# poyentung/ebsd-vae

Measured on AMD Instinct MI355X. Metric: EBSD patterns/sec (128x128, fwd+bwd), higher is better.
Workload: dtype fp32 I/O, f16x3 split MFMA; 1 GPU; c2: VariationalAutoEncoderRawData 128x128, latent 16, batch 256/GPU, fwd+loss+bwd+Adam; global_batch=256, image_size=128, latent_dim=16, parallelism=dp1

## Files before the change

### ebsd-vae_amd/csrc/conv_split.hip

```cpp
#include "conv_common.h"
#include "instnorm_fin.h"

#include <stdlib.h>
#include <type_traits>

namespace ev {

static_assert(NP_F16 == EBSDVAE_PIECES_F16, "piece-format id");

#ifdef EV_PIPE_TRACE
__device__ unsigned long long ev_pipe_trace[4096 * 8 * 6];
#define EV_T(x) unsigned long long x = __builtin_amdgcn_s_memtime()
#define EV_TACC(acc, t0) acc += __builtin_amdgcn_s_memtime() - t0
#else
#define EV_T(x)
#define EV_TACC(acc, t0)
#endif


typedef __bf16 bf16x8 __attribute__((ext_vector_type(8)));
typedef __bf16 bf16x4 __attribute__((ext_vector_type(4)));

constexpr int XCK = 8;
constexpr int ACT_FIRST = 5;
// ... 268 lines not shown

EV_DEVINL void pipe_barrier_lds() {
  asm volatile("" ::: "memory");
  __builtin_amdgcn_s_waitcnt(0xF | (7 << 4) | (3 << 14));
  __builtin_amdgcn_s_barrier();
  asm volatile("" ::: "memory");
}

template <int N>
EV_DEVINL void pipe_barrier() {
  static_assert(N >= 0 && N < 16, "vmcnt range");
  asm volatile("" ::: "memory");
  __builtin_amdgcn_s_waitcnt(N | (7 << 4));
  __builtin_amdgcn_s_barrier();
  asm volatile("" ::: "memory");
}

#ifndef EV_EPI_POL
#define EV_EPI_POL 2
#endif
constexpr int kEpiPol = EV_EPI_POL;

template <int MF, int NF, int FP>
constexpr bool pipe_prefetch_ok() { return NF == 1 && (FP == P_ID || FP == FP_UPSUM); }
template <int MF, int NF, int FP>
constexpr int pipe_prefetch_n() {
  return pipe_prefetch_ok<MF, NF, FP>() ? (FP == FP_UPSUM ? 8 * (MF / 2) : 16 * MF) : 1;
}
template <int MF, int NF, int FP, int NT, int PH = 0>
EV_DEVINL void pipe_epilogue(f32x16 (&acc)[MF][NF], const float* __restrict__ bias,
                             float* __restrict__ y, float2* __restrict__ spart, int H, int W, int b0,
                             int h0, int wpx0, int mfs, int slot, int co_base, int hk, int l32,
                             const float* __restrict__ yprev, const float2* __restrict__ stprev,
                             double2* __restrict__ ipart, float* __restrict__ ypool, float sc,
                             float (&pv)[pipe_prefetch_n<MF, NF, FP>()]) {
  static_assert(MF % 2 == 0, "fragments in 64-pixel pairs");
  static_assert(PH == 0 || pipe_prefetch_ok<MF, NF, FP>(), "prefetch phases: NF 1, P_ID / UPSUM");
  constexpr int NG = MF / 2;
  constexpr bool FUSED = FP == P_ID || FP == P_POOL || FP == P_UP || FP == FP_UPSUM;
#ifndef EV_EPI_OPAQUE
#define EV_EPI_OPAQUE 1
#endif
  constexpr bool EPI_OPAQUE = EV_EPI_OPAQUE && FP == FP_POOLOUT;
  if constexpr (PH == 1) {
    const int nf = 0;
    const int co = co_base + l32;
    if constexpr (FP == FP_UPSUM) {
      const int W2 = W >> 1;
      const auto rp = __builtin_amdgcn_make_buffer_rsrc(
          (void*)(yprev + ((size_t)b0 * (H >> 1) + (h0 >> 1)) * W2 * NT), 0, 0x7fffffff, 0x00020000);
#pragma unroll
      for (int g = 0; g < NG; ++g) {
        const int m0 = 2 * g;
#pragma unroll
        for (int k = 0; k < 8; ++k) {
// ... 80 lines not shown
            gs[k] = (acc[m0][nf][r] + acc[m0][nf][r + 1]) + (acc[m0 + 1][nf][r] + acc[m0 + 1][nf][r + 1]);
            prow = (wpx0 / W + m0) >> 1;
            pc = ((wpx0 % W + 4 * hk) >> 1) + (((r & 3) + 8 * (r >> 2)) >> 1);
          } else {
            const int mf = m0 + (k >> 2), r = 2 * (k & 3);
            gs[k] = (acc[mf][nf][r] + acc[mf][nf][r + 1]) + (acc[mf][nf][r + 8] + acc[mf][nf][r + 9]);
            prow = (wpx0 + mf * mfs) / W >> 1;
            pc = ((r & 3) + 8 * (r >> 2) + 4 * hk) >> 1;
          }
          off[k] = ((prow * W2 + pc) * NT + co) * 4;
        }
#pragma unroll
        for (int k = 0; k < 8; ++k)
          v[k] = PH == 2 ? pv[g * 8 + k]
                         : __builtin_bit_cast(float, __builtin_amdgcn_raw_buffer_load_b32(rp, off[k], 0, kEpiPol));
        float s1 = 0.f, s2 = 0.f;
#pragma unroll
        for (int k = 0; k < 8; ++k) {
          const float h = inbwd_acc<P_ID>(gs[k], &v[k], sp, spc, s1, s2);
          __builtin_amdgcn_raw_buffer_store_b32(__builtin_bit_cast(unsigned, h), rq, off[k], 0, kEpiPol);
        }
        s1 += __shfl_xor(s1, 32, 64);
        s2 += __shfl_xor(s2, 32, 64);
        if (hk == 0) ipart[((size_t)b0 * T + slot + g) * NT + co] = make_double2((double)s1, (double)s2);
      }
    }
    if (FP == FP_POOLOUT) {
      const int W2 = W >> 1;
      const auto rq = __builtin_amdgcn_make_buffer_rsrc(
          (void*)(ypool + ((size_t)b0 * (H >> 1) + (h0 >> 1)) * W2 * NT), 0, 0x7fffffff, 0x00020000);
#pragma unroll
      for (int m0 = 0; m0 < MF; m0 += 2) {
        if (W >= 32) {
          const int prow = (wpx0 / W + m0) >> 1, pcol = (wpx0 % W + 4 * hk) >> 1;
          int pb = ((prow * W2 + pcol) * NT + co) * 4;
          if constexpr (EPI_OPAQUE) asm volatile("" : "+v"(pb));
#pragma unroll
          for (int r = 0; r < 16; r += 2) {
            const float m = fmaxf(fmaxf(acc[m0][nf][r], acc[m0][nf][r + 1]),
                                  fmaxf(acc[m0 + 1][nf][r], acc[m0 + 1][nf][r + 1]));
            const int dc = ((r & 3) + 8 * (r >> 2)) >> 1;
            __builtin_amdgcn_raw_buffer_store_b32(__builtin_bit_cast(unsigned, m), rq,
                                                  pb + dc * NT * 4, 0, kEpiPol);
          }
        } else {
#pragma unroll
          for (int mf = m0; mf < m0 + 2; ++mf) {
// ... 28 lines not shown
#pragma unroll
        for (int e0 = 32 * g; e0 < 32 * g + 32; e0 += G) {
          float v[G][NL];
#pragma unroll
          for (int j = 0; j < G; ++j) {
            const int e = e0 + j, mf = e >> 4, r = e & 15;
            const int pl = pbase + mf * 32 + (r & 3) + 8 * (r >> 2);
#pragma unroll
            for (int k = 0; k < NL; ++k)
              v[j][k] = PH == 2 ? pv[e]
                                : __builtin_bit_cast(float, __builtin_amdgcn_raw_buffer_load_b32(
                                                                rp, (inbwd_pix<FP>(pl, W, lW, k) * NT + co) * 4, 0, kEpiPol));
          }
#pragma unroll
          for (int j = 0; j < G; ++j) {
            const int e = e0 + j, mf = e >> 4, r = e & 15;
            const float h = inbwd_acc<FP>(acc[mf][nf][r], v[j], sp, spc, s1, s2);
            __builtin_amdgcn_raw_buffer_store_b32(__builtin_bit_cast(unsigned, h), ry,
                                                  vbase + (mf * mfs + (r & 3) + 8 * (r >> 2)) * NT * 4, 0, kEpiPol);
          }
        }
        s1 += __shfl_xor(s1, 32, 64);
        s2 += __shfl_xor(s2, 32, 64);
        if (hk == 0) ipart[((size_t)b0 * T + slot + g) * NT + co] = make_double2((double)s1, (double)s2);
      }
    }
    if (!FUSED && spart) {
#pragma unroll
      for (int g = 0; g < NG; ++g) {
        float sg = s[g];
        sg += __shfl_xor(sg, 32, 64);
        const float mean = sg * (1.0f / 64);
        float q = 0.f;
#pragma unroll
        for (int mf = 2 * g; mf < 2 * g + 2; ++mf)
#pragma unroll
          for (int r = 0; r < 16; ++r) {
            const float d = acc[mf][nf][r] - mean;
            q = fmaf(d, d, q);
          }
        q += __shfl_xor(q, 32, 64);
        if (hk == 0) spart[((size_t)b0 * T + slot + g) * NT + co] = make_float2(mean, q);
      }
    }
  }
}

#ifndef EV_WREG
#define EV_WREG 1
#endif
constexpr bool pipe_wreg(int NWV, int WM, int NF, int NI, int WR) {
  return EV_WREG && NWV == 4 && WM == 1 && NF == 1 && NI == 1 && WR == 0;
}

template <int NP, int NWV, int WM, int MF, int NF, int KX, int MODE, int FP, int NI, int WR>
__global__ __launch_bounds__(NWV * 64, (MODE == ACT_FIRST || pipe_wreg(NWV, WM, NF, NI, WR)) ? 1 : 2) void conv3x3_pipe_kernel(
    const float* __restrict__ src, const float2* __restrict__ sstats, const char* __restrict__ wp,
    const float* __restrict__ bias, float* __restrict__ y, float2* __restrict__ spart,
    float* __restrict__ act_out, int B, int H, int W, int Cin, int TH, int tpb,
    const float* __restrict__ yprev, const float2* __restrict__ stprev, double2* __restrict__ ipart,
    float* __restrict__ ypool, const float* __restrict__ gmax, int gmT, float2* __restrict__ st_out,
    float2* __restrict__ bst_out, double fin_inv_hw, const float* __restrict__ w0,
    const float* __restrict__ b0) {
  constexpr int WN = NWV / WM;
  constexpr int NT = WN * NF * 32;
// ... 15 lines not shown
  static_assert(!FIRST || (WR > 0 && NI == 1), "ACT_FIRST: the resident-weight single-image form");
  extern __shared__ __attribute__((aligned(16))) char xsm[];
  const int HP = TH + 2, WP = W + 2;
  const int pixI = HP * WP;
  const int pixP = NI * pixI;
  const int xslab = (pixP + 1) * XPS;
  char* lw0 = xsm;
  char* lx0 = xsm + (WR ? WR * WSLAB : 2 * WSLABP);
  const int XTS = FIRST ? (TH + 4) * (W + 2) : 0;
  float* xtl = reinterpret_cast<float*>(lx0 + 2 * xslab);
  const float4* wtab = reinterpret_cast<const float4*>(xtl + 2 * XTS);

  const int tid = threadIdx.x, lane = tid & 63, wave = tid >> 6;
  const int wm = wave % WM, wn = wave / WM;
  const int l32 = lane & 31, hk = lane >> 5;
  const int tpi = H / TH;
  const int tpx = TH * W;
  const int nch = Cin / XCK;
  const int t0 = blockIdx.x * tpb;
  const int ntl = min(tpb, ((B + NI - 1) / NI) * tpi - t0);
  const int nit = ntl * nch;

  int fpx0 = wm * MW, mfs = 32;
  if ((FP == FP_POOLOUT || FP == FP_UPSUM) && W >= 32) {
    const int cbs = W >> 5, rp = wm / cbs;
    fpx0 = MF * rp * W + (wm - rp * cbs) * 32;
    mfs = W;
  }
  int abase[MF];
#pragma unroll
  for (int mf = 0; mf < MF; ++mf) {
    const int p = fpx0 + mf * mfs + l32;
    const int im = p / tpx, pr = p - im * tpx;
    const int r = pr / W, c = pr - r * W;
    abase[mf] = im * pixI + r * WP + c;
  }
  int toff[5];
#pragma unroll
  for (int s = 0; s < 5; ++s) {
    const int t = min(2 * s + hk, 8);
    toff[s] = (t / 3) * WP + t % 3;
  }

  const int Hs = POOL ? 2 * H : (UPS ? H / 2 : H);
  const int Ws = POOL ? 2 * W : (UPS ? W / 2 : W);
  const int q = tid & 1;
  constexpr int WPI = NWV / NI;
  static_assert(NWV % NI == 0, "waves split evenly over the tile's images");
  const int img_w = wave / WPI;
  const int tig = tid - img_w * WPI * 64;
// ... 227 lines not shown
    }
  };

  f32x16 acc[MF][NF];
  auto zero_acc = [&]() EV_LAMBDA_INLINE {
#pragma unroll
    for (int mf = 0; mf < MF; ++mf)
#pragma unroll
      for (int nf = 0; nf < NF; ++nf)
#pragma unroll
        for (int r = 0; r < 16; ++r) acc[mf][nf][r] = 0.f;
  };
  const int ncol = wn * NF * 32 + l32;
#ifdef EV_PIPE_NOPREF
  constexpr bool PREF = false;
#else
  constexpr bool PREF = pipe_prefetch_ok<MF, NF, FP>() && NI == 1;
#endif
  float pv[pipe_prefetch_n<MF, NF, FP>()];
  auto epi_prefetch = [&](int it) EV_LAMBDA_INLINE {
    int b0, h0, ch;
    coords(it, b0, h0, ch);
    pipe_epilogue<MF, NF, FP, NT, PREF ? 1 : 0>(acc, bias, y, spart, H, W, b0, h0, fpx0, mfs, 0,
                                                wn * NF * 32, hk, l32, yprev, stprev, ipart, ypool, 1.f, pv);
  };
  auto epilogue = [&](int it_done, f32x16 (&ea)[MF][NF]) EV_LAMBDA_INLINE {
    int b0, h0, ch;
    coords(it_done, b0, h0, ch);
    const int im = NI == 1 ? 0 : (wm * MW) / tpx;
    const int wpx0 = fpx0 - im * tpx;
    float sc = 1.f;
    if constexpr (NP == NP_F16) {
      sc = ldexpf(1.f, -wshift);
      if constexpr (GS) sc = ldexpf(sc, -gshift(min(b0 + im, B - 1)));
    }
#ifdef EV_PIPE_NOEPI
    if (sc == 12345.f)
#else
    if (NI == 1 || b0 + im < B)
#endif
      pipe_epilogue<MF, NF, FP, NT, PREF ? 2 : 0>(ea, bias, y, spart, H, W, b0 + im, h0, wpx0, mfs,
                                                  (h0 * W + wm * MW - im * tpx) / 64, wn * NF * 32, hk,
                                                  l32, yprev, stprev, ipart, ypool, sc, pv);
  };

#ifdef EV_PIPE_TRACE
  unsigned long long tr_issue = 0, tr_k = 0, tr_bar = 0, tr_epi = 0;
  const unsigned long long tr_start = __builtin_amdgcn_s_memtime();
  const unsigned long long tr_rstart = __builtin_amdgcn_s_memrealtime();
#endif
  auto body = [&](int it, auto P_c) EV_LAMBDA_INLINE {
    constexpr int P = decltype(P_c)::value;
    constexpr int SL_LD = PD == 2 ? P : 0;
    constexpr int SL_ST = PD == 2 ? 1 - P : 0;
    EV_T(tb0);
    const int it1 = min(it + 1, nit - 1), itp = min(it + PD, nit - 1);
    if constexpr (PREF && P == 1)
      if ((it & (nch - 1)) == nch - 1) epi_prefetch(it);
#ifndef EV_PIPE_LATE_ISSUE
    issue_weights(it1, lw0 + (1 - P) * WSLABP);
    if constexpr (WREG) issue_wreg(it1, std::integral_constant<int, WREG ? 1 - P : 0>());
    issue_halo(itp, std::integral_constant<int, SL_LD>());
#endif
    EV_TACC(tr_issue, tb0);
    EV_T(tb1);
// ... 168 lines not shown
      if (item_live(k)) stage_item(std::integral_constant<int, 0>(), k, fs, lx0);
    stage_post(std::integral_constant<int, 0>(), fs, lx0);
  }
  if constexpr (WR) {
    asm volatile("s_waitcnt vmcnt(%0)" ::"n"(NLD) : "memory");
  }
  __syncthreads();
  for (int tl = 0; tl < ntl; ++tl) {
    for (int ch = 0; ch < nch; ch += 2) {
      body(tl * nch + ch, std::integral_constant<int, 0>());
      body(tl * nch + ch + 1, std::integral_constant<int, 1>());
    }
    EV_T(te0);
    epilogue(tl * nch, acc);
    zero_acc();
    EV_TACC(tr_epi, te0);
  }
  if (st_out || bst_out) {
    asm volatile("s_waitcnt vmcnt(0)" ::: "memory");
    __threadfence_block();
    __syncthreads();
    const int tpi = NI == 1 ? H / TH : 1;
    const int g0 = t0 / tpi, g1 = (t0 + ntl - 1) / tpi;
    for (int gi = g0; gi <= g1; ++gi)
      for (int im = 0; im < NI; ++im) {
        const int b = gi * NI + im;
        if (b >= B) break;
        if (st_out)
          in_stats_finalize_image(spart, st_out, NT, (H * W) / 64, 64.f, b, tid,
                                  reinterpret_cast<float*>(xsm));
        if (bst_out)
          in_bwd_finalize_image(ipart, bst_out, NT, (H * W) / 64, fin_inv_hw, b, tid,
                                reinterpret_cast<double*>(xsm));
      }
  }
#ifdef EV_PIPE_TRACE
  if (lane == 0 && blockIdx.x < 4096) {
    unsigned long long* o = ev_pipe_trace + ((size_t)blockIdx.x * 8 + (wave & 7)) * 6;
    o[0] = __builtin_amdgcn_s_memtime() - tr_start;
    o[1] = tr_issue; o[2] = tr_k; o[3] = tr_bar; o[4] = tr_epi;
    o[5] = __builtin_amdgcn_s_memrealtime() - tr_rstart;
  }
#endif
}

__global__ __launch_bounds__(256) void pack_wmax_kernel(const PackBatch pb) {
  const ebsdvae_pack_desc& q = pb.d[blockIdx.y];
  const int n = q.cin * q.cout * 9;
  float m = 0.f;
  for (int i = blockIdx.x * 256 + threadIdx.x; i < n; i += kF16MaxParts * 256) m = fmaxf(m, fabsf(q.src[i]));
  for (int off = 32; off > 0; off >>= 1) m = fmaxf(m, __shfl_xor(m, off));
  __shared__ float wm[4];
  if ((threadIdx.x & 63) == 0) wm[threadIdx.x >> 6] = m;
  __syncthreads();
  if (threadIdx.x == 0) {
// ... 66 lines not shown
  static const bool v = [] {
    const char* e = getenv("EBSDVAE_CONV_SMALL1");
    return !(e && e[0] == '0');
  }();
  return v;
}

static bool use_multi_image() {
  static const int v = [] {
    const char* e = getenv("EBSDVAE_CONV_MULTI_IMAGE");
    return (e && e[0] == '0') ? 0 : 1;
  }();
  return v != 0;
}

static bool use_wres() {
  static const bool v = [] {
    const char* e = getenv("EBSDVAE_WRES");
    return !(e && e[0] == '0');
  }();
  return v;
}

static int cu_count(hipStream_t s) {
  if (const int n = evh::stream_cus(s)) return n;
  static int cache[64] = {0};
  int dev = 0;
  (void)hipGetDevice(&dev);
  if (dev < 0 || dev >= 64) dev = 0;
  if (!cache[dev]) {
    int n = 0;
    if (hipDeviceGetAttribute(&n, hipDeviceAttributeMultiprocessorCount, dev) != hipSuccess || n <= 0) n = 256;
    cache[dev] = n;
  }
  return cache[dev];
}

struct X3Cfg {
  int M, TH, NT, KX, nwv;
  int NI;
  int wr;
  size_t lds;
  size_t lds_pipe;
};

static bool plan_split(int H, int W, int cin, int cout, int np, X3Cfg* c) {
  if ((np != 2 && np != 3 && np != NP_F16) || cin % (2 * XCK) || !(cout == 128 || cout == 64 || cout == 32)) return false;
  if (np == NP_F16 && !use_pipe()) return false;
  auto pow2 = [](int v) { return v > 0 && (v & (v - 1)) == 0; };
  if (!pow2(cin / XCK) || !pow2(H) || !pow2(W)) return false;
  if (!ev_buf_bytes_ok(4LL * H * W * (cin > cout ? cin : cout) * 4)) return false;
  c->M = (np != 2 && cout != 128) ? 512 : 256;
  c->NI = 1;
  c->NT = cout;
  c->nwv = (cout == 128 || np != 2) ? 8 : 4;
  if (H * W < c->M) {
    if (!((np == 3 || np == NP_F16) && cout == 128 && H * W == 64 && use_pipe() && use_multi_image()))
      return false;
    c->M = 128;
    c->NI = 2;
    c->TH = H;
    if (np == NP_F16 && use_small_one_image()) {
      c->M = 64;
      c->NI = 1;
      c->nwv = 4;
    }
  } else {
    if (W > c->M || c->M % W) return false;
    c->TH = c->M / W;
    if (H % c->TH) return false;
  }
  const int pixI = (c->TH + 2) * (W + 2);
  const int pix = c->NI * pixI;
  const int tpg = (c->nwv / c->NI) * 64;
  c->KX = use_pipe() ? ((c->TH + 2) * W * 2 + tpg - 1) / tpg : (pixI * 2 + tpg - 1) / tpg;
  const int kxmax = np == 2 ? (cout == 128 ? 2 : (cout == 64 ? 5 : 7))
                            : (np == NP_F16 ? (cout == 128 ? 2 : (cout == 64 ? 3 : 4))
                                            : (cout == 128 ? 2 : (cout == 64 ? 4 : 5)));
  if (c->KX > kxmax) return false;
  const int wslab = XTAPS * npc(np) * cout * 16;
  c->lds = 2 * (size_t)wslab + 2 * (size_t)(pix + 1) * XPS;
  c->lds_pipe = 2 * (size_t)pipe_dma_per(wslab, c->nwv) * c->nwv * 1024 + 2 * (size_t)(pix + 1) * XPS;
  if (c->lds_pipe > 160 * 1024) c->lds_pipe = 0;
  c->wr = 0;
  const size_t lds_wr = 4 * (size_t)wslab + 2 * (size_t)(pix + 1) * XPS;
  if (np == NP_F16 && cin == 4 * XCK && c->NI == 1 && use_wres() && use_pipe() && lds_wr <= 160 * 1024) {
    c->wr = 4;
    c->lds_pipe = lds_wr;
  }
  if (c->NI > 1 || np == NP_F16) return c->lds_pipe != 0;
  return c->lds <= 160 * 1024;
}

static bool pipe_owns_images(const X3Cfg& c, int B, int H, hipStream_t s) {
  static const bool on = [] {
    const char* e = getenv("EBSDVAE_FUSE_FINALIZE");
    return !(e && e[0] == '0');
  }();
  if (!on || !(c.NI > 1 || (use_pipe() && c.lds_pipe))) return false;
  const int tpi = c.NI > 1 ? 1 : H / c.TH;
  const int ntiles = ((B + c.NI - 1) / c.NI) * tpi;
  const int ncu = cu_count(s);
  const int tpb = (ntiles + ncu - 1) / ncu;
  return tpb % tpi == 0;
}

static size_t first_lds_extra(int TH, int W) {
  return (2 * (size_t)(TH + 4) * (W + 2) + FIRST_WTAB) * sizeof(float);
}
// ... 38 lines not shown
                      const float* bias, float* y, float* part, float* aout, int B, int H, int W,
                      int cin, hipStream_t s, int pmode, const InBwdFuse& f) {
  if (pmode >= 0) {
    switch (pmode) {
      case P_ID: launch_x3_1<NP, NWV, WM, MF, NF, KX, ACT_RAW, P_ID, NI, WR>(c, src, nullptr, wp, nullptr, y, nullptr, nullptr, B, H, W, cin, s, f); break;
      case P_POOL: launch_x3_1<NP, NWV, WM, MF, NF, KX, ACT_RAW, P_POOL, NI, WR>(c, src, nullptr, wp, nullptr, y, nullptr, nullptr, B, H, W, cin, s, f); break;
      case P_UPSUM:
        if constexpr (NI == 1)
          launch_x3_1<NP, NWV, WM, MF, NF, KX, ACT_RAW, FP_UPSUM, NI, WR>(c, src, nullptr, wp, nullptr, y, nullptr, nullptr, B, H, W, cin, s, f);
        break;
      default: launch_x3_1<NP, NWV, WM, MF, NF, KX, ACT_RAW, P_UP, NI, WR>(c, src, nullptr, wp, nullptr, y, nullptr, nullptr, B, H, W, cin, s, f); break;
    }
    return;
  }
  if constexpr (NI == 1) {
    if (f.ypool) {
      launch_x3_1<NP, NWV, WM, MF, NF, KX, ACT_NORM, FP_POOLOUT, NI, WR>(c, src, st, wp, bias, y, part, aout, B, H, W, cin, s, f);
      return;
    }
  }
  switch (mode) {
    case ACT_RAW: launch_x3_1<NP, NWV, WM, MF, NF, KX, ACT_RAW, FP_NONE, NI, WR>(c, src, st, wp, bias, y, part, aout, B, H, W, cin, s, f); break;
    case ACT_NORM: launch_x3_1<NP, NWV, WM, MF, NF, KX, ACT_NORM, FP_NONE, NI, WR>(c, src, st, wp, bias, y, part, aout, B, H, W, cin, s, f); break;
    case ACT_NORM_POOL: launch_x3_1<NP, NWV, WM, MF, NF, KX, ACT_NORM_POOL, FP_NONE, NI, 0>(c, src, st, wp, bias, y, part, aout, B, H, W, cin, s, f); break;
    case ACT_UP: launch_x3_1<NP, NWV, WM, MF, NF, KX, ACT_UP, FP_NONE, NI, WR>(c, src, st, wp, bias, y, part, aout, B, H, W, cin, s, f); break;
    default: launch_x3_1<NP, NWV, WM, MF, NF, KX, ACT_NORM_UP, FP_NONE, NI, WR>(c, src, st, wp, bias, y, part, aout, B, H, W, cin, s, f); break;
  }
}

static void dispatch_split(const X3Cfg& c, int np, const float* src, const float* st, int mode,
                           const void* wp, const float* bias, float* y, float* part, float* aout,
                           int B, int H, int W, int cin, int cout, hipStream_t s, int pmode,
                           const InBwdFuse& f) {
  if (np == 2) {
    if (cout == 128)
      launch_x3<2, 8, 4, 2, 2, 2>(c, src, st, mode, wp, bias, y, part, aout, B, H, W, cin, s, pmode, f);
    else if (cout == 64)
      launch_x3<2, 4, 4, 2, 2, 5>(c, src, st, mode, wp, bias, y, part, aout, B, H, W, cin, s, pmode, f);
    else
      launch_x3<2, 4, 4, 2, 1, 7>(c, src, st, mode, wp, bias, y, part, aout, B, H, W, cin, s, pmode, f);
  } else if (np == NP_F16) {
    if (cout == 128 && c.NI > 1)
      launch_x3<NP_F16, 8, 2, 2, 1, 1, 2>(c, src, st, mode, wp, bias, y, part, aout, B, H, W, cin, s, pmode, f);
    else if (cout == 128 && c.M == 64)
      launch_x3<NP_F16, 4, 1, 2, 1, 1>(c, src, st, mode, wp, bias, y, part, aout, B, H, W, cin, s, pmode, f);
    else if (cout == 128)
      launch_x3<NP_F16, 8, 4, 2, 2, 2>(c, src, st, mode, wp, bias, y, part, aout, B, H, W, cin, s, pmode, f);
    else if (cout == 64 && c.wr)
      launch_x3<NP_F16, 8, 8, 2, 2, 3, 1, 4>(c, src, st, mode, wp, bias, y, part, aout, B, H, W, cin, s, pmode, f);
    else if (cout == 64)
      launch_x3<NP_F16, 8, 8, 2, 2, 3>(c, src, st, mode, wp, bias, y, part, aout, B, H, W, cin, s, pmode, f);
    else if (c.KX <= 3 && c.wr)
      launch_x3<NP_F16, 8, 8, 2, 1, 3, 1, 4>(c, src, st, mode, wp, bias, y, part, aout, B, H, W, cin, s, pmode, f);
    else if (c.KX <= 3)
      launch_x3<NP_F16, 8, 8, 2, 1, 3>(c, src, st, mode, wp, bias, y, part, aout, B, H, W, cin, s, pmode, f);
    else if (c.wr)
      launch_x3<NP_F16, 8, 8, 2, 1, 4, 1, 4>(c, src, st, mode, wp, bias, y, part, aout, B, H, W, cin, s, pmode, f);
    else
      launch_x3<NP_F16, 8, 8, 2, 1, 4>(c, src, st, mode, wp, bias, y, part, aout, B, H, W, cin, s, pmode, f);
  } else {
    if (cout == 128 && c.NI > 1)
      launch_x3<3, 8, 2, 2, 1, 1, 2>(c, src, st, mode, wp, bias, y, part, aout, B, H, W, cin, s, pmode, f);
    else if (cout == 128)
      launch_x3<3, 8, 4, 2, 2, 2>(c, src, st, mode, wp, bias, y, part, aout, B, H, W, cin, s, pmode, f);
    else if (cout == 64)
      launch_x3<3, 8, 8, 2, 2, 4>(c, src, st, mode, wp, bias, y, part, aout, B, H, W, cin, s, pmode, f);
    else
      launch_x3<3, 8, 8, 2, 1, 5>(c, src, st, mode, wp, bias, y, part, aout, B, H, W, cin, s, pmode, f);
  }
}

}

using namespace ev;

#ifdef EV_PIPE_TRACE
extern "C" int ebsdvae_debug_pipe_trace(void* host, size_t bytes) {
  if (bytes > sizeof(ev_pipe_trace)) bytes = sizeof(ev_pipe_trace);
  return hipMemcpyFromSymbol(host, HIP_SYMBOL(ev_pipe_trace), bytes, 0, hipMemcpyDeviceToHost) == hipSuccess ? 0 : 1;
}
#endif

extern "C" int ebsdvae_conv3x3_split_supported(int H, int W, int cin, int cout, int pieces) {
  X3Cfg c;
  return plan_split(H, W, cin, cout, pieces, &c) ? 1 : 0;
}

extern "C" int ebsdvae_conv3x3_split_stat_tiles(int H, int W, int cout) {
  (void)cout;
  if (!ev_dim_ok(H) || !ev_dim_ok(W)) return -1;
  return (H * W) / 64;
}

extern "C" size_t ebsdvae_pack_split_bytes(int cin, int cout, int pieces) {
  if (cin <= 0 || cout <= 0 || !(pieces == 2 || pieces == 3 || pieces == NP_F16)) return 0;
  return (size_t)(cin / XCK) * XTAPS * npc(pieces) * cout * XCK * 2 +
         (pieces == NP_F16 ? kF16PackTrailer : 0);
}

extern "C" int ebsdvae_pack_conv_weights_split(const ebsdvae_pack_desc* descs, int n, int pieces,
                                               ebsdvae_stream_t stream) {
  EV_REQUIRE(descs && n > 0 && n <= EBSDVAE_MAX_PACK, "pack_conv_weights_split: n=%d out of range", n);
  EV_REQUIRE(pieces == 2 || pieces == 3 || pieces == NP_F16,
             "pack_conv_weights_split: pieces=%d (2, 3 or %d)", pieces, NP_F16);
  PackBatch pb;
// ... 4 lines not shown
    EV_REQUIRE(q.src && q.dst && q.cin > 0 && q.cout > 0 && (q.kind == 0 || q.kind == 1) && ci_ % XCK == 0,
               "pack_conv_weights_split: bad descriptor %d", i);
    pb.d[i] = q;
    const int e = (ci_ / XCK) * XTAPS * (q.for_dgrad ? q.cin : q.cout) * XCK;
    if (e > maxn) maxn = e;
  }
  int bx = (maxn + 255) / 256;
  if (bx > 64) bx = 64;
  if (pieces == NP_F16)
    hipLaunchKernelGGL(pack_wmax_kernel, dim3(kF16MaxParts, n), dim3(256), 0, (hipStream_t)stream, pb);
  hipLaunchKernelGGL(pack_split_kernel, dim3(bx, n), dim3(256), 0, (hipStream_t)stream, pb, pieces);
  return evh::check_launch("pack_conv_weights_split");
}

extern "C" int ebsdvae_conv3x3_fwd_split(const float* src, const float* src_stats, int src_mode,
                                         const void* wpack, const float* bias, float* y,
                                         float* stat_part, float* act_out, int B, int H, int W,
                                         int cin, int cout, int pieces, ebsdvae_stream_t stream) {
  X3Cfg c;
  EV_REQUIRE(src && wpack && y && B > 0, "conv3x3_fwd_split: null pointer or empty batch");
  EV_REQUIRE(src_mode >= 0 && src_mode <= 4, "conv3x3_fwd_split: bad src_mode %d", src_mode);
  EV_REQUIRE(src_mode == ACT_RAW || src_mode == ACT_UP || src_stats,
             "conv3x3_fwd_split: NORM modes need src_stats");
  EV_REQUIRE(plan_split(H, W, cin, cout, pieces, &c),
             "conv3x3_fwd_split: unsupported shape H=%d W=%d cin=%d cout=%d pieces=%d", H, W, cin, cout,
             pieces);
  dispatch_split(c, pieces, src, src_stats, src_mode, wpack, bias, y, stat_part, act_out, B, H, W,
                 cin, cout, (hipStream_t)stream, -1, InBwdFuse());
  return evh::check_launch("conv3x3_fwd_split");
}

extern "C" int ebsdvae_conv3x3_split_pool_ok(int H, int W, int cin, int cout, int pieces) {
  X3Cfg c;
  return (plan_split(H, W, cin, cout, pieces, &c) && use_pipe() && c.lds_pipe && c.NI == 1 &&
          c.TH % 2 == 0 && W >= 16 && (W & (W - 1)) == 0) ? 1 : 0;
}

extern "C" int ebsdvae_conv3x3_fwd_split_pooled(const float* src, const float* src_stats,
                                                int src_mode, const void* wpack, const float* bias,
                                                float* y, float* ypool, float* stat_part, int B,
                                                int H, int W, int cin, int cout, int pieces,
                                                ebsdvae_stream_t stream) {
  X3Cfg c;
  EV_REQUIRE(src && src_stats && wpack && y && ypool && stat_part && B > 0,
             "conv3x3_fwd_split_pooled: null pointer or empty batch");
  EV_REQUIRE(src_mode == ACT_NORM, "conv3x3_fwd_split_pooled: src_mode %d (ACT_NORM only)", src_mode);
  EV_REQUIRE(ebsdvae_conv3x3_split_pool_ok(H, W, cin, cout, pieces) && plan_split(H, W, cin, cout, pieces, &c),
             "conv3x3_fwd_split_pooled: unsupported shape H=%d W=%d cin=%d cout=%d pieces=%d", H, W,
             cin, cout, pieces);
  InBwdFuse f;
  f.ypool = ypool;
  dispatch_split(c, pieces, src, src_stats, src_mode, wpack, bias, y, stat_part, nullptr, B, H, W,
                 cin, cout, (hipStream_t)stream, -1, f);
  return evh::check_launch("conv3x3_fwd_split_pooled");
}

extern "C" int ebsdvae_conv3x3_dgrad_inbwd_split(const float* g, const void* wpack, float* gin,
                                                 const float* y_prev, const float* st_prev,
                                                 int pmode, double* part, int B, int H, int W,
                                                 int cin, int cout, int pieces,
                                                 ebsdvae_stream_t stream) {
  X3Cfg c;
  EV_REQUIRE(g && wpack && gin && B > 0, "conv3x3_dgrad_inbwd_split: null pointer or empty batch");
  EV_REQUIRE(pieces != NP_F16, "conv3x3_dgrad_inbwd_split: fp16 pieces need the gradient scale "
             "(ebsdvae_conv3x3_dgrad_inbwd_f16)");
  EV_REQUIRE(pmode >= -1 && pmode <= P_UPSUM, "conv3x3_dgrad_inbwd_split: bad pmode %d", pmode);
  EV_REQUIRE(pmode != P_UPSUM || ebsdvae_conv3x3_split_pool_ok(H, W, cin, cout, pieces),
             "conv3x3_dgrad_inbwd_split: summed upsample adjoint unsupported for H=%d W=%d", H, W);
  EV_REQUIRE(pmode < 0 || (y_prev && st_prev && part && (W & (W - 1)) == 0),
             "conv3x3_dgrad_inbwd_split: fused reduce needs y_prev, st_prev, part and W = 2^k");
// ... 2 lines not shown
             cin, cout, pieces);
  InBwdFuse f;
  f.yprev = y_prev;
  f.stprev = (const float2*)st_prev;
  f.part = (double2*)part;
  dispatch_split(c, pieces, g, nullptr, ACT_RAW, wpack, nullptr, gin, nullptr, nullptr, B, H, W, cin,
                 cout, (hipStream_t)stream, pmode, f);
  return evh::check_launch("conv3x3_dgrad_inbwd_split");
}

extern "C" int ebsdvae_conv3x3_dgrad_inbwd_f16(const float* g, const float* gmax, int gm_tiles,
                                               const void* wpack, float* gin, const float* y_prev,
                                               const float* st_prev, int pmode, double* part, int B,
                                               int H, int W, int cin, int cout,
                                               ebsdvae_stream_t stream) {
  X3Cfg c;
  EV_REQUIRE(g && gmax && gm_tiles > 0 && wpack && gin && B > 0,
             "conv3x3_dgrad_inbwd_f16: null pointer, empty batch or no gradient maxima");
  EV_REQUIRE(pmode >= -1 && pmode <= P_UPSUM, "conv3x3_dgrad_inbwd_f16: bad pmode %d", pmode);
  EV_REQUIRE(pmode != P_UPSUM || ebsdvae_conv3x3_split_pool_ok(H, W, cin, cout, NP_F16),
             "conv3x3_dgrad_inbwd_f16: summed upsample adjoint unsupported for H=%d W=%d", H, W);
  EV_REQUIRE(pmode < 0 || (y_prev && st_prev && part && (W & (W - 1)) == 0),
             "conv3x3_dgrad_inbwd_f16: fused reduce needs y_prev, st_prev, part and W = 2^k");
  EV_REQUIRE(plan_split(H, W, cin, cout, NP_F16, &c),
             "conv3x3_dgrad_inbwd_f16: unsupported shape H=%d W=%d cin=%d cout=%d", H, W, cin, cout);
  InBwdFuse f;
  f.yprev = y_prev;
  f.stprev = (const float2*)st_prev;
  f.part = (double2*)part;
  f.gmax = gmax;
  f.gmT = gm_tiles;
  dispatch_split(c, NP_F16, g, nullptr, ACT_RAW, wpack, nullptr, gin, nullptr, nullptr, B, H, W, cin,
                 cout, (hipStream_t)stream, pmode, f);
  return evh::check_launch("conv3x3_dgrad_inbwd_f16");
}

extern "C" int ebsdvae_conv3x3_fwd_split_st(const float* src, const float* src_stats, int src_mode,
                                            const void* wpack, const float* bias, float* y,
                                            float* ypool, float* stat_part, float* st, int B,
                                            int H, int W, int cin, int cout, int pieces,
                                            ebsdvae_stream_t stream) {
  X3Cfg c;
  EV_REQUIRE(src && wpack && (y || ypool) && stat_part && st && B > 0,
             "conv3x3_fwd_split_st: null pointer or empty batch");
  EV_REQUIRE(src_mode >= 0 && src_mode <= 4, "conv3x3_fwd_split_st: bad src_mode %d", src_mode);
  EV_REQUIRE(src_mode == ACT_RAW || src_mode == ACT_UP || src_stats,
             "conv3x3_fwd_split_st: NORM modes need src_stats");
  EV_REQUIRE(!ypool || (src_mode == ACT_NORM && ebsdvae_conv3x3_split_pool_ok(H, W, cin, cout, pieces)),
             "conv3x3_fwd_split_st: pooled output unsupported for H=%d W=%d src_mode=%d", H, W, src_mode);
  EV_REQUIRE(plan_split(H, W, cin, cout, pieces, &c),
             "conv3x3_fwd_split_st: unsupported shape H=%d W=%d cin=%d cout=%d pieces=%d", H, W, cin,
             cout, pieces);
  const bool fused = pipe_owns_images(c, B, H, (hipStream_t)stream);
  InBwdFuse f;
  f.ypool = ypool;
  if (fused) f.st_out = (float2*)st;
  dispatch_split(c, pieces, src, src_stats, src_mode, wpack, bias, y, stat_part, nullptr, B, H, W,
                 cin, cout, (hipStream_t)stream, -1, f);
  if (int rc = evh::check_launch("conv3x3_fwd_split_st")) return rc;
  if (fused) return 0;
  const int T = ebsdvae_conv3x3_split_stat_tiles(H, W, cout);
  return ebsdvae_in_stats_finalize(stat_part, st, B, cout, T, (H * W) / T, stream);
}

extern "C" int ebsdvae_conv3x3_dgrad_inbwd_f16_bst(const float* g, const float* gmax, int gm_tiles,
                                                   const void* wpack, float* gin, const float* y_prev,
                                                   const float* st_prev, int pmode, double* part,
                                                   float* bst, int prev_hw, int B, int H, int W,
                                                   int cin, int cout, ebsdvae_stream_t stream) {
  X3Cfg c;
  EV_REQUIRE(g && gmax && gm_tiles > 0 && wpack && gin && B > 0,
             "conv3x3_dgrad_inbwd_f16_bst: null pointer, empty batch or no gradient maxima");
  EV_REQUIRE(pmode >= 0 && pmode <= P_UPSUM && y_prev && st_prev && part && bst && prev_hw > 0 &&
                 (W & (W - 1)) == 0,
             "conv3x3_dgrad_inbwd_f16_bst: fused reduce needs pmode >= 0, y_prev, st_prev, part, bst, "
             "prev_hw and W = 2^k");
  EV_REQUIRE(pmode != P_UPSUM || ebsdvae_conv3x3_split_pool_ok(H, W, cin, cout, NP_F16),
             "conv3x3_dgrad_inbwd_f16_bst: summed upsample adjoint unsupported for H=%d W=%d", H, W);
  EV_REQUIRE(plan_split(H, W, cin, cout, NP_F16, &c),
             "conv3x3_dgrad_inbwd_f16_bst: unsupported shape H=%d W=%d cin=%d cout=%d", H, W, cin, cout);
  const bool fused = pipe_owns_images(c, B, H, (hipStream_t)stream);
  InBwdFuse f;
  f.yprev = y_prev;
  f.stprev = (const float2*)st_prev;
  f.part = (double2*)part;
  f.gmax = gmax;
  f.gmT = gm_tiles;
  if (fused) {
    f.bst_out = (float2*)bst;
    f.inv_hw = 1.0 / (double)prev_hw;
  }
  dispatch_split(c, NP_F16, g, nullptr, ACT_RAW, wpack, nullptr, gin, nullptr, nullptr, B, H, W, cin,
                 cout, (hipStream_t)stream, pmode, f);
  if (int rc = evh::check_launch("conv3x3_dgrad_inbwd_f16_bst")) return rc;
  if (fused) return 0;
  return ebsdvae_in_bwd_finalize(part, bst, B, cout, ebsdvae_conv3x3_split_stat_tiles(H, W, cout), prev_hw,
                                 stream);
}

extern "C" int ebsdvae_conv3x3_fwd_split_first_ok(int H, int W, int cin, int cout, int pieces) {
  X3Cfg c;
  if (pieces != NP_F16 || cin != 4 * XCK || cout != 32 || !plan_split(H, W, cin, cout, pieces, &c))
// ... 44 lines not shown
```

### ebsd-vae_amd/latice/_native.py

```python
from __future__ import annotations

import ctypes
import os
import threading

import torch

_HERE = os.path.dirname(os.path.abspath(__file__))
LIB_PATH = os.environ.get(
    "EBSDVAE_LIB", os.path.join(os.path.dirname(_HERE), "lib", "libebsdvae.so"))

P = ctypes.c_void_p
I = ctypes.c_int
I64 = ctypes.c_int64
U64 = ctypes.c_uint64
F = ctypes.c_float

SIGNATURES = {
    "ebsdvae_last_error": [],
    "ebsdvae_version": [],
    "ebsdvae_stream_wait": [P, P],
    "ebsdvae_fork_arm": [P],
    "ebsdvae_fork_wait": [P, P],
    "ebsdvae_stream_create_cus": [I, I, P],
    "ebsdvae_stream_destroy_cus": [P],
    "ebsdvae_conv_first_stat_tiles": [I, I],
    "ebsdvae_conv_first_fwd": [P, P, P, P, P, I, I, I, I, P],
    "ebsdvae_conv_first_stats": [P, P, P, P, I, I, I, I, P],
    "ebsdvae_in_bwd_first_apply_wgrad_rc": [P, P, P, P, P, P, P, P, I, I, I, I, P],
    "ebsdvae_in_bwd_first_happly_wgrad_rc": [P, P, P, P, P, P, P, P, I, I, I, I, P],
    "ebsdvae_in_bwd_first_happly_wgrad": [P, P, P, P, P, P, P, I, I, I, I, P],
    "ebsdvae_pack_conv_weight": [P, P, I, I, I, I, P],
    "ebsdvae_pack_conv_weights": [P, I, P],
    "ebsdvae_conv3x3_fwd": [P, P, I, P, P, P, P, P, I, I, I, I, I, P],
    "ebsdvae_conv3x3_stat_tiles": [I, I, I],
    "ebsdvae_conv3x3_dgrad_inbwd": [P, P, P, P, P, I, P, I, I, I, I, I, P],
    "ebsdvae_conv3x3_split_supported": [I, I, I, I, I],
    "ebsdvae_conv3x3_split_stat_tiles": [I, I, I],
    "ebsdvae_pack_split_bytes": [I, I, I],
    "ebsdvae_pack_conv_weights_split": [P, I, I, P],
    "ebsdvae_conv3x3_fwd_split": [P, P, I, P, P, P, P, P, I, I, I, I, I, I, P],
    "ebsdvae_conv3x3_split_pool_ok": [I, I, I, I, I],
    "ebsdvae_conv3x3_fwd_split_pooled": [P, P, I, P, P, P, P, P, I, I, I, I, I, I, P],
    "ebsdvae_conv3x3_dgrad_inbwd_split": [P, P, P, P, P, I, P, I, I, I, I, I, I, P],
    "ebsdvae_conv3x3_dgrad_inbwd_f16": [P, P, I, P, P, P, P, I, P, I, I, I, I, I, P],
    "ebsdvae_conv3x3_fwd_split_st": [P, P, I, P, P, P, P, P, P, I, I, I, I, I, I, P],
    "ebsdvae_conv3x3_fwd_split_first_ok": [I, I, I, I, I],
    "ebsdvae_conv3x3_fwd_split_first": [P, P, P, P, P, P, P, P, P, P, I, I, I, I, I, I, P],
    "ebsdvae_conv3x3_dgrad_inbwd_f16_bst": [P, P, I, P, P, P, P, I, P, P, I, I, I, I, I, I, P],
    "ebsdvae_conv3x3_cout1_fwd": [P, P, I, P, P, P, I, I, I, I, I, P],
    "ebsdvae_conv3x3_cout1_dgrad": [P, P, P, I, I, I, I, P],
    "ebsdvae_conv3x3_wgrad_slices": [I, I, I, I, I],
    "ebsdvae_conv3x3_wgrad": [P, P, I, P, P, P, I, I, I, I, I, P],
    "ebsdvae_conv3x3_wgrad_split_slices": [I, I, I, I, I, I],
    "ebsdvae_conv3x3_wgrad_split": [P, P, I, P, P, P, I, I, I, I, I, I, P],
    "ebsdvae_conv3x3_wgrad_f16": [P, P, I, P, P, I, P, P, I, I, I, I, I, P],
    "ebsdvae_conv3x3_dwgrad_slices": [I, I, I, I, I],
    "ebsdvae_conv3x3_dwgrad_stat_tiles": [I, I],
    "ebsdvae_conv3x3_dwgrad_f16": [P, P, I, P, P, P, I, P, P, P, P, I, I, I, I, I, P],
    "ebsdvae_wgrad_reduce_work": [I, I, I],
    "ebsdvae_wgrad_reduce": [P, P, I, P, P, I, I, I, P, P],
# ... 142 lines not shown
```

### include/ebsdvae.h

```cpp
#ifndef EBSDVAE_H_
#define EBSDVAE_H_

#include <stddef.h>
#include <stdint.h>

#ifdef __cplusplus
extern "C" {
#endif

typedef void* ebsdvae_stream_t;

const char* ebsdvae_last_error(void);
#define EBSDVAE_ABI_VERSION 2
int ebsdvae_version(void);

int ebsdvae_stream_wait(ebsdvae_stream_t waiter, ebsdvae_stream_t signaler);
int ebsdvae_fork_arm(ebsdvae_stream_t signaler);
int ebsdvae_fork_wait(ebsdvae_stream_t waiter, ebsdvae_stream_t signaler);
int ebsdvae_stream_create_cus(int first, int count, ebsdvae_stream_t* out);
int ebsdvae_stream_destroy_cus(ebsdvae_stream_t stream);

int ebsdvae_pack_conv_weight(const float* src, float* dst, int cin, int cout, int kind,
                             int for_dgrad, ebsdvae_stream_t stream);

// ... 11 lines not shown
                        ebsdvae_stream_t stream);
int ebsdvae_conv3x3_stat_tiles(int H, int W, int cout);

int ebsdvae_conv3x3_dgrad_inbwd(const float* g, const float* wpack, float* gin,
                                const float* y_prev, const float* st_prev, int pmode,
                                double* part, int B, int H, int W, int cin, int cout,
                                ebsdvae_stream_t stream);

int ebsdvae_conv_first_stat_tiles(int H, int W);
int ebsdvae_conv_first_stats(const float* x, const float* w0, const float* b0, float* st, int B,
                             int H, int W, int C, ebsdvae_stream_t stream);

int ebsdvae_conv_first_fwd(const float* x, const float* w0, const float* b0, float* y,
                           float* part, int B, int H, int W, int C, ebsdvae_stream_t stream);
int ebsdvae_conv3x3_cout1_fwd(const float* src, const float* src_stats, int src_mode,
                              const float* w, const float* bias, float* out, int flip,
                              int B, int H, int W, int cin, ebsdvae_stream_t stream);
int ebsdvae_conv3x3_cout1_dgrad(const float* g, const float* w, float* gin, int B, int H,
                                int W, int cin, ebsdvae_stream_t stream);

#define EBSDVAE_PIECES_F16 16
int ebsdvae_conv3x3_split_supported(int H, int W, int cin, int cout, int pieces);
int ebsdvae_conv3x3_split_stat_tiles(int H, int W, int cout);
size_t ebsdvae_pack_split_bytes(int cin, int cout, int pieces);
int ebsdvae_pack_conv_weights_split(const ebsdvae_pack_desc* descs, int n, int pieces,
                                    ebsdvae_stream_t stream);
int ebsdvae_conv3x3_fwd_split(const float* src, const float* src_stats, int src_mode,
                              const void* wpack, const float* bias, float* y, float* stat_part,
                              float* act_out, int B, int H, int W, int cin, int cout, int pieces,
                              ebsdvae_stream_t stream);
int ebsdvae_conv3x3_split_pool_ok(int H, int W, int cin, int cout, int pieces);
int ebsdvae_conv3x3_fwd_split_pooled(const float* src, const float* src_stats, int src_mode,
                                     const void* wpack, const float* bias, float* y, float* ypool,
                                     float* stat_part, int B, int H, int W, int cin, int cout,
                                     int pieces, ebsdvae_stream_t stream);
int ebsdvae_conv3x3_dgrad_inbwd_split(const float* g, const void* wpack, float* gin,
                                      const float* y_prev, const float* st_prev, int pmode,
                                      double* part, int B, int H, int W, int cin, int cout,
                                      int pieces, ebsdvae_stream_t stream);
int ebsdvae_conv3x3_dgrad_inbwd_f16(const float* g, const float* gmax, int gm_tiles,
                                    const void* wpack, float* gin, const float* y_prev,
                                    const float* st_prev, int pmode, double* part, int B, int H,
                                    int W, int cin, int cout, ebsdvae_stream_t stream);
int ebsdvae_conv3x3_fwd_split_st(const float* src, const float* src_stats, int src_mode,
                                 const void* wpack, const float* bias, float* y, float* ypool,
                                 float* stat_part, float* st, int B, int H, int W, int cin,
// ... 186 lines not shown
```

Measured before the change: 30160 patterns/s.

## Add tall 1024-pixel tile config for cout=32 split convs on upsample paths

Adds a 'tall' plan for the f16-split pipelined conv3x3 when cout is 32 and width is 128 or 64. It uses M=1024 pixel tiles with MF=4 fragments per wave and a larger KX limit, and adjusts the stat-slot indexing (slot_w, gss stride) and the finalize thread index so per-64-pixel statistics still land in the right slots. By default it is enabled only for W=128, cin=64 forward convs in upsample modes, with an env var and API toggle to override. The intent is more weight reuse and fewer tiles per image, at the cost of more registers and LDS and the loss of weight-resident mode for those shapes.

```diff
diff --git a/ebsd-vae_amd/csrc/conv_split.hip b/ebsd-vae_amd/csrc/conv_split.hip
--- a/ebsd-vae_amd/csrc/conv_split.hip
+++ b/ebsd-vae_amd/csrc/conv_split.hip
@@ -314,7 +314,7 @@
 constexpr int kEpiPol = EV_EPI_POL;
 
 template <int MF, int NF, int FP>
-constexpr bool pipe_prefetch_ok() { return NF == 1 && (FP == P_ID || FP == FP_UPSUM); }
+constexpr bool pipe_prefetch_ok() { return NF == 1 && ((FP == P_ID && MF <= 2) || FP == FP_UPSUM); }
 template <int MF, int NF, int FP>
 constexpr int pipe_prefetch_n() {
   return pipe_prefetch_ok<MF, NF, FP>() ? (FP == FP_UPSUM ? 8 * (MF / 2) : 16 * MF) : 1;
@@ -322,7 +322,7 @@
 template <int MF, int NF, int FP, int NT, int PH = 0>
 EV_DEVINL void pipe_epilogue(f32x16 (&acc)[MF][NF], const float* __restrict__ bias,
                              float* __restrict__ y, float2* __restrict__ spart, int H, int W, int b0,
-                             int h0, int wpx0, int mfs, int slot, int co_base, int hk, int l32,
+                             int h0, int wpx0, int mfs, int slot, int gss, int co_base, int hk, int l32,
                              const float* __restrict__ yprev, const float2* __restrict__ stprev,
                              double2* __restrict__ ipart, float* __restrict__ ypool, float sc,
                              float (&pv)[pipe_prefetch_n<MF, NF, FP>()]) {
@@ -449,7 +449,7 @@
         }
         s1 += __shfl_xor(s1, 32, 64);
         s2 += __shfl_xor(s2, 32, 64);
-        if (hk == 0) ipart[((size_t)b0 * T + slot + g) * NT + co] = make_double2((double)s1, (double)s2);
+        if (hk == 0) ipart[((size_t)b0 * T + slot + g * gss) * NT + co] = make_double2((double)s1, (double)s2);
       }
     }
     if (FP == FP_POOLOUT) {
@@ -524,7 +524,7 @@
         }
         s1 += __shfl_xor(s1, 32, 64);
         s2 += __shfl_xor(s2, 32, 64);
-        if (hk == 0) ipart[((size_t)b0 * T + slot + g) * NT + co] = make_double2((double)s1, (double)s2);
+        if (hk == 0) ipart[((size_t)b0 * T + slot + g * gss) * NT + co] = make_double2((double)s1, (double)s2);
       }
     }
     if (!FUSED && spart) {
@@ -542,7 +542,7 @@
             q = fmaf(d, d, q);
           }
         q += __shfl_xor(q, 32, 64);
-        if (hk == 0) spart[((size_t)b0 * T + slot + g) * NT + co] = make_float2(mean, q);
+        if (hk == 0) spart[((size_t)b0 * T + slot + g * gss) * NT + co] = make_float2(mean, q);
       }
     }
   }
@@ -604,10 +604,13 @@
   const int nit = ntl * nch;
 
   int fpx0 = wm * MW, mfs = 32;
+  int slot_w = (wm * MW) / 64, gss = 1;
   if ((FP == FP_POOLOUT || FP == FP_UPSUM) && W >= 32) {
     const int cbs = W >> 5, rp = wm / cbs;
     fpx0 = MF * rp * W + (wm - rp * cbs) * 32;
     mfs = W;
+    slot_w = (MF / 2) * rp * cbs + (wm - rp * cbs);
+    gss = cbs;
   }
   int abase[MF];
 #pragma unroll
@@ -881,7 +884,7 @@
     int b0, h0, ch;
     coords(it, b0, h0, ch);
     pipe_epilogue<MF, NF, FP, NT, PREF ? 1 : 0>(acc, bias, y, spart, H, W, b0, h0, fpx0, mfs, 0,
-                                                wn * NF * 32, hk, l32, yprev, stprev, ipart, ypool, 1.f, pv);
+                                                1, wn * NF * 32, hk, l32, yprev, stprev, ipart, ypool, 1.f, pv);
   };
   auto epilogue = [&](int it_done, f32x16 (&ea)[MF][NF]) EV_LAMBDA_INLINE {
     int b0, h0, ch;
@@ -899,7 +902,7 @@
     if (NI == 1 || b0 + im < B)
 #endif
       pipe_epilogue<MF, NF, FP, NT, PREF ? 2 : 0>(ea, bias, y, spart, H, W, b0 + im, h0, wpx0, mfs,
-                                                  (h0 * W + wm * MW - im * tpx) / 64, wn * NF * 32, hk,
+                                                  (h0 * W - im * tpx) / 64 + slot_w, gss, wn * NF * 32, hk,
                                                   l32, yprev, stprev, ipart, ypool, sc, pv);
   };
 
@@ -1114,15 +1117,17 @@
     __syncthreads();
     const int tpi = NI == 1 ? H / TH : 1;
     const int g0 = t0 / tpi, g1 = (t0 + ntl - 1) / tpi;
+    const int ftid = MF > 2 ? wave_u * 64 + (int)__builtin_amdgcn_mbcnt_hi(~0u, __builtin_amdgcn_mbcnt_lo(~0u, 0u))
+                            : tid;
     for (int gi = g0; gi <= g1; ++gi)
       for (int im = 0; im < NI; ++im) {
         const int b = gi * NI + im;
         if (b >= B) break;
         if (st_out)
-          in_stats_finalize_image(spart, st_out, NT, (H * W) / 64, 64.f, b, tid,
+          in_stats_finalize_image(spart, st_out, NT, (H * W) / 64, 64.f, b, ftid,
                                   reinterpret_cast<float*>(xsm));
         if (bst_out)
-          in_bwd_finalize_image(ipart, bst_out, NT, (H * W) / 64, fin_inv_hw, b, tid,
+          in_bwd_finalize_image(ipart, bst_out, NT, (H * W) / 64, fin_inv_hw, b, ftid,
                                 reinterpret_cast<double*>(xsm));
       }
   }
@@ -1235,6 +1240,16 @@
   return v;
 }
 
+constexpr int TALL_AUTO = -1;
+static int g_conv_tall = -2;
+static int tall_setting() {
+  static const int v = [] {
+    const char* e = getenv("EBSDVAE_CONV_TALL");
+    return (e && e[0] == '0') ? 0 : ((e && e[0] == '1') ? 1 : TALL_AUTO);
+  }();
+  return g_conv_tall == -2 ? v : g_conv_tall;
+}
+
 static int cu_count(hipStream_t s) {
   if (const int n = evh::stream_cus(s)) return n;
   static int cache[64] = {0};
@@ -1257,13 +1272,21 @@
   size_t lds_pipe;
 };
 
-static bool plan_split(int H, int W, int cin, int cout, int np, X3Cfg* c) {
+static bool plan_split(int H, int W, int cin, int cout, int np, X3Cfg* c, int tall_mode = -1) {
   if ((np != 2 && np != 3 && np != NP_F16) || cin % (2 * XCK) || !(cout == 128 || cout == 64 || cout == 32)) return false;
   if (np == NP_F16 && !use_pipe()) return false;
   auto pow2 = [](int v) { return v > 0 && (v & (v - 1)) == 0; };
   if (!pow2(cin / XCK) || !pow2(H) || !pow2(W)) return false;
   if (!ev_buf_bytes_ok(4LL * H * W * (cin > cout ? cin : cout) * 4)) return false;
   c->M = (np != 2 && cout != 128) ? 512 : 256;
+  bool tall = tall_mode >= 0 && tall_mode != ACT_NORM_POOL && use_pipe() && np == NP_F16 &&
+              cout == 32 && (W == 128 || W == 64) && H % (1024 / W) == 0;
+  if (tall) {
+    const int ts = tall_setting();
+    const bool measured = W == 128 && cin == 8 * XCK && (tall_mode == ACT_UP || tall_mode == ACT_NORM_UP);
+    tall = ts == 1 || (ts == TALL_AUTO && measured);
+  }
+  if (tall) c->M = 1024;
   c->NI = 1;
   c->NT = cout;
   c->nwv = (cout == 128 || np != 2) ? 8 : 4;
@@ -1288,7 +1311,7 @@
   const int tpg = (c->nwv / c->NI) * 64;
   c->KX = use_pipe() ? ((c->TH + 2) * W * 2 + tpg - 1) / tpg : (pixI * 2 + tpg - 1) / tpg;
   const int kxmax = np == 2 ? (cout == 128 ? 2 : (cout == 64 ? 5 : 7))
-                            : (np == NP_F16 ? (cout == 128 ? 2 : (cout == 64 ? 3 : 4))
+                            : (np == NP_F16 ? (cout == 128 ? 2 : (cout == 64 ? 3 : (tall ? 5 : 4)))
                                             : (cout == 128 ? 2 : (cout == 64 ? 4 : 5)));
   if (c->KX > kxmax) return false;
   const int wslab = XTAPS * npc(np) * cout * 16;
@@ -1297,7 +1320,7 @@
   if (c->lds_pipe > 160 * 1024) c->lds_pipe = 0;
   c->wr = 0;
   const size_t lds_wr = 4 * (size_t)wslab + 2 * (size_t)(pix + 1) * XPS;
-  if (np == NP_F16 && cin == 4 * XCK && c->NI == 1 && use_wres() && use_pipe() && lds_wr <= 160 * 1024) {
+  if (np == NP_F16 && cin == 4 * XCK && c->NI == 1 && !tall && use_wres() && use_pipe() && lds_wr <= 160 * 1024) {
     c->wr = 4;
     c->lds_pipe = lds_wr;
   }
@@ -1382,7 +1405,10 @@
   switch (mode) {
     case ACT_RAW: launch_x3_1<NP, NWV, WM, MF, NF, KX, ACT_RAW, FP_NONE, NI, WR>(c, src, st, wp, bias, y, part, aout, B, H, W, cin, s, f); break;
     case ACT_NORM: launch_x3_1<NP, NWV, WM, MF, NF, KX, ACT_NORM, FP_NONE, NI, WR>(c, src, st, wp, bias, y, part, aout, B, H, W, cin, s, f); break;
-    case ACT_NORM_POOL: launch_x3_1<NP, NWV, WM, MF, NF, KX, ACT_NORM_POOL, FP_NONE, NI, 0>(c, src, st, wp, bias, y, part, aout, B, H, W, cin, s, f); break;
+    case ACT_NORM_POOL:
+      if constexpr (MF <= 2)
+        launch_x3_1<NP, NWV, WM, MF, NF, KX, ACT_NORM_POOL, FP_NONE, NI, 0>(c, src, st, wp, bias, y, part, aout, B, H, W, cin, s, f);
+      break;
     case ACT_UP: launch_x3_1<NP, NWV, WM, MF, NF, KX, ACT_UP, FP_NONE, NI, WR>(c, src, st, wp, bias, y, part, aout, B, H, W, cin, s, f); break;
     default: launch_x3_1<NP, NWV, WM, MF, NF, KX, ACT_NORM_UP, FP_NONE, NI, WR>(c, src, st, wp, bias, y, part, aout, B, H, W, cin, s, f); break;
   }
@@ -1410,6 +1436,8 @@
       launch_x3<NP_F16, 8, 8, 2, 2, 3, 1, 4>(c, src, st, mode, wp, bias, y, part, aout, B, H, W, cin, s, pmode, f);
     else if (cout == 64)
       launch_x3<NP_F16, 8, 8, 2, 2, 3>(c, src, st, mode, wp, bias, y, part, aout, B, H, W, cin, s, pmode, f);
+    else if (c.M == 1024)
+      launch_x3<NP_F16, 8, 8, 4, 1, 5>(c, src, st, mode, wp, bias, y, part, aout, B, H, W, cin, s, pmode, f);
     else if (c.KX <= 3 && c.wr)
       launch_x3<NP_F16, 8, 8, 2, 1, 3, 1, 4>(c, src, st, mode, wp, bias, y, part, aout, B, H, W, cin, s, pmode, f);
     else if (c.KX <= 3)
@@ -1441,6 +1469,11 @@
 }
 #endif
 
+extern "C" int ebsdvae_set_conv_tall(int on) {
+  g_conv_tall = on < 0 ? -2 : (on != 0);
+  return 0;
+}
+
 extern "C" int ebsdvae_conv3x3_split_supported(int H, int W, int cin, int cout, int pieces) {
   X3Cfg c;
   return plan_split(H, W, cin, cout, pieces, &c) ? 1 : 0;
@@ -1491,7 +1524,7 @@
   EV_REQUIRE(src_mode >= 0 && src_mode <= 4, "conv3x3_fwd_split: bad src_mode %d", src_mode);
   EV_REQUIRE(src_mode == ACT_RAW || src_mode == ACT_UP || src_stats,
              "conv3x3_fwd_split: NORM modes need src_stats");
-  EV_REQUIRE(plan_split(H, W, cin, cout, pieces, &c),
+  EV_REQUIRE(plan_split(H, W, cin, cout, pieces, &c, src_mode),
              "conv3x3_fwd_split: unsupported shape H=%d W=%d cin=%d cout=%d pieces=%d", H, W, cin, cout,
              pieces);
   dispatch_split(c, pieces, src, src_stats, src_mode, wpack, bias, y, stat_part, act_out, B, H, W,
@@ -1514,7 +1547,7 @@
   EV_REQUIRE(src && src_stats && wpack && y && ypool && stat_part && B > 0,
              "conv3x3_fwd_split_pooled: null pointer or empty batch");
   EV_REQUIRE(src_mode == ACT_NORM, "conv3x3_fwd_split_pooled: src_mode %d (ACT_NORM only)", src_mode);
-  EV_REQUIRE(ebsdvae_conv3x3_split_pool_ok(H, W, cin, cout, pieces) && plan_split(H, W, cin, cout, pieces, &c),
+  EV_REQUIRE(ebsdvae_conv3x3_split_pool_ok(H, W, cin, cout, pieces) && plan_split(H, W, cin, cout, pieces, &c, src_mode),
              "conv3x3_fwd_split_pooled: unsupported shape H=%d W=%d cin=%d cout=%d pieces=%d", H, W,
              cin, cout, pieces);
   InBwdFuse f;
@@ -1563,7 +1596,7 @@
              "conv3x3_dgrad_inbwd_f16: summed upsample adjoint unsupported for H=%d W=%d", H, W);
   EV_REQUIRE(pmode < 0 || (y_prev && st_prev && part && (W & (W - 1)) == 0),
              "conv3x3_dgrad_inbwd_f16: fused reduce needs y_prev, st_prev, part and W = 2^k");
-  EV_REQUIRE(plan_split(H, W, cin, cout, NP_F16, &c),
+  EV_REQUIRE(plan_split(H, W, cin, cout, NP_F16, &c, ACT_RAW),
              "conv3x3_dgrad_inbwd_f16: unsupported shape H=%d W=%d cin=%d cout=%d", H, W, cin, cout);
   InBwdFuse f;
   f.yprev = y_prev;
@@ -1589,7 +1622,7 @@
              "conv3x3_fwd_split_st: NORM modes need src_stats");
   EV_REQUIRE(!ypool || (src_mode == ACT_NORM && ebsdvae_conv3x3_split_pool_ok(H, W, cin, cout, pieces)),
              "conv3x3_fwd_split_st: pooled output unsupported for H=%d W=%d src_mode=%d", H, W, src_mode);
-  EV_REQUIRE(plan_split(H, W, cin, cout, pieces, &c),
+  EV_REQUIRE(plan_split(H, W, cin, cout, pieces, &c, src_mode),
              "conv3x3_fwd_split_st: unsupported shape H=%d W=%d cin=%d cout=%d pieces=%d", H, W, cin,
              cout, pieces);
   const bool fused = pipe_owns_images(c, B, H, (hipStream_t)stream);
@@ -1618,7 +1651,7 @@
              "prev_hw and W = 2^k");
   EV_REQUIRE(pmode != P_UPSUM || ebsdvae_conv3x3_split_pool_ok(H, W, cin, cout, NP_F16),
              "conv3x3_dgrad_inbwd_f16_bst: summed upsample adjoint unsupported for H=%d W=%d", H, W);
-  EV_REQUIRE(plan_split(H, W, cin, cout, NP_F16, &c),
+  EV_REQUIRE(plan_split(H, W, cin, cout, NP_F16, &c, ACT_RAW),
              "conv3x3_dgrad_inbwd_f16_bst: unsupported shape H=%d W=%d cin=%d cout=%d", H, W, cin, cout);
   const bool fused = pipe_owns_images(c, B, H, (hipStream_t)stream);
   InBwdFuse f;
diff --git a/ebsd-vae_amd/latice/_native.py b/ebsd-vae_amd/latice/_native.py
--- a/ebsd-vae_amd/latice/_native.py
+++ b/ebsd-vae_amd/latice/_native.py
@@ -37,6 +37,7 @@
     "ebsdvae_conv3x3_dgrad_inbwd": [P, P, P, P, P, I, P, I, I, I, I, I, P],
     "ebsdvae_conv3x3_split_supported": [I, I, I, I, I],
     "ebsdvae_conv3x3_split_stat_tiles": [I, I, I],
+    "ebsdvae_set_conv_tall": [I],
     "ebsdvae_pack_split_bytes": [I, I, I],
     "ebsdvae_pack_conv_weights_split": [P, I, I, P],
     "ebsdvae_conv3x3_fwd_split": [P, P, I, P, P, P, P, P, I, I, I, I, I, I, P],
diff --git a/include/ebsdvae.h b/include/ebsdvae.h
--- a/include/ebsdvae.h
+++ b/include/ebsdvae.h
@@ -57,6 +57,7 @@
 #define EBSDVAE_PIECES_F16 16
 int ebsdvae_conv3x3_split_supported(int H, int W, int cin, int cout, int pieces);
 int ebsdvae_conv3x3_split_stat_tiles(int H, int W, int cout);
+int ebsdvae_set_conv_tall(int on);
 size_t ebsdvae_pack_split_bytes(int cin, int cout, int pieces);
 int ebsdvae_pack_conv_weights_split(const ebsdvae_pack_desc* descs, int n, int pieces,
                                     ebsdvae_stream_t stream);
```

Measured after the change: 30170 patterns/s, median of 2. Within noise of the previous version (+0.0%).
